# Grandediw/Unmanned_Aerial_Vehicles

Hardware: AMD Instinct MI355X
Metric: GP predictions/sec (mean+var) at N_train=65536, D=9 (higher is better)
Workload: dtype f32; 1 GPU; C3: N_train=65536, D=9, P=3, batched predict mean+var over 10000 query points per GPU per step (horizon 20 x 500 rollouts), fp32 predict on an fp64 factor; n_train=65536, features=9, outputs=3, parallelism=query-sharded x1, model replicated (every rank fits redundantly)

## Files before the change

### include/gpk.h

```cpp
#ifndef GPK_H
#define GPK_H

#include <stddef.h>
#include <stdint.h>

#ifdef __cplusplus
extern "C" {
#endif

typedef struct gpk_context* gpk_handle;

#define GPK_API __attribute__((visibility("default")))

enum { GPK_F32 = 0, GPK_F64 = 1 };
enum { GPK_OK = 0, GPK_NOT_PD = 1, GPK_BAD_ARG = 2, GPK_HIP_ERROR = 3 };
enum { GPK_TILE = 128, GPK_MAX_D = 64, GPK_MAX_D_PREDICT = 16, GPK_MAX_P = 16, GPK_MAX_BATCH = 8 };

GPK_API int gpk_create(gpk_handle* h, int device);
GPK_API void gpk_destroy(gpk_handle h);
GPK_API const char* gpk_last_error(gpk_handle h);
#define GPK_OWN_STREAM ((void*)(intptr_t)-1)
GPK_API int gpk_set_stream(gpk_handle h, void* stream);
GPK_API int gpk_synchronize(gpk_handle h);
GPK_API int64_t gpk_padded(int64_t n);
// ... 25 lines not shown

GPK_API int gpk_factor_to_f32(gpk_handle h, const double* L, int64_t Np, int64_t ldl, const double* winv,
                      float* Lf, int64_t ldlf, float* winvf);

GPK_API int gpk_potrs(gpk_handle h, const double* L, int64_t Np, int64_t ldl, const double* winv,
              const double* Y, int64_t N, int P, double* alpha);

GPK_API int gpk_potrs_inv(gpk_handle h, const double* W, int64_t Np, int64_t ldw, const double* Y, int64_t N,
                  int P, double* alpha);

GPK_API int gpk_trsm_lower_left(gpk_handle h, int dtype, const void* L, int64_t Np, int64_t ldl,
                        const void* winv, void* B, int64_t Mp, int64_t ldb);
GPK_API int gpk_colsumsq(gpk_handle h, int dtype, const void* B, int64_t Np, int64_t Mp, int64_t ldb,
                 double* out);

GPK_API int gpk_predict_mean(gpk_handle h, int dtype, const void* X, const void* alpha, int64_t N, int D,
                     int P, const double* ls, double sf2, const double* y_mean,
                     const double* y_std, const void* Xq, int64_t M, void* mean);

#define GPK_HOST_MAX_M 4096
GPK_API int gpk_predict_host(gpk_handle h, const double* X, const double* alpha, int64_t N, int D, int P,
                     const double* ls, double sf2, const double* y_mean, const double* y_std,
                     const double* W, int64_t Np, int64_t ldw, double kss, double floor_,
                     const double* Xq_host, int64_t M, double* mean_host, double* var_host);

GPK_API int gpk_predict_host_multi(gpk_handle h, int B, const double* const* X, const double* const* alpha, int64_t N, int D,
                           const double* ls, const double* sf2, const double* y_mean, const double* y_std,
                           const double* const* W, int64_t Np, int64_t ldw, const double* kss, double floor_,
                           const double* Xq_host, int64_t M, double* mean_host, double* var_host);

GPK_API int gpk_predict_mean_mfma(gpk_handle h, const float* X, const float* alpha, int64_t N, int D, int P,
                          const double* ls, double sf2, const double* center, const double* y_mean,
                          const double* y_std, const float* Xq, int64_t M, float* mean);

GPK_API int gpk_split3(gpk_handle h, const float* src, int64_t rows, int64_t cols, int64_t ld, void* dst);
GPK_API int gpk_predict_var_inv_split(gpk_handle h, const float* X, int64_t N, int D, const double* ls, double sf2,
                              const void* W3, int64_t Np, const float* Xq, int64_t M, double kss, double floor_,
                              float* work, void* work3, double* var);

GPK_API int gpk_split2_rows(gpk_handle h, const float* W, int64_t n, int64_t ld, float* scales, void* dst);
GPK_API int gpk_split2_rows_f64(gpk_handle h, const double* W, int64_t n, int64_t ld, float* scales, void* dst);
GPK_API int gpk_split2_rows_f64_absmax(gpk_handle h, const double* W, int64_t n, int64_t ld, float* scales, void* dst);
GPK_API int gpk_predict_var_inv_split2(gpk_handle h, const float* X, int64_t N, int D, const double* ls, double sf2,
                                       const void* W2, const float* w_scales, int64_t Np, const float* Xq, int64_t M,
                                       double kss, double floor_, void* work2, double* var);

GPK_API int gpk_predict_mean_var_split2(gpk_handle h, const float* X, const float* alpha, int64_t N, int D, int P,
                                        const double* ls, double sf2, const double* center, const double* y_mean,
                                        const double* y_std, const void* W2, const float* w_scales, int64_t Np,
                                        const float* Xq, int64_t M, double kss, double floor_, void* work2,
                                        float* mean_tmp, double recheck_below, unsigned* low_count, double* out);
GPK_API int gpk_pack_mean_var(gpk_handle h, int dtype, const void* mean, const double* var, int64_t M, int P,
                              const double* y_std, double* out);

GPK_API int gpk_predict_mean_multi(gpk_handle h, int dtype, const void* X, const void* alpha, int64_t N, int D,
                           int B, const double* ls, const double* sf2, const double* y_mean,
                           const double* y_std, const void* Xq, int64_t M, void* mean);

GPK_API int gpk_predict_var(gpk_handle h, int dtype, const void* X, int64_t N, int D, const double* ls,
                    double sf2, const void* L, int64_t Np, int64_t ldl, const void* winv,
                    const void* Xq, int64_t M, double kss, double floor, void* work,
                    double* var);

GPK_API int gpk_trtri(gpk_handle h, const double* L, int64_t Np, int64_t ldl, const double* winv, double* W,
              int64_t ldw, double* work);
GPK_API int gpk_trtri_absmax(gpk_handle h, const double* L, int64_t Np, int64_t ldl, const double* winv, double* W,
              int64_t ldw, double* work, float* block_absmax);
GPK_API int gpk_tril_to_f32(gpk_handle h, const double* A, int64_t Np, int64_t lda, float* Af, int64_t ldaf);
GPK_API int gpk_predict_var_inv(gpk_handle h, int dtype, const void* X, int64_t N, int D, const double* ls,
                        double sf2, const void* W, int64_t Np, int64_t ldw, const void* Xq, int64_t M,
                        double kss, double floor, void* work, double* var);

GPK_API int gpk_predict_cov_inv(gpk_handle h, int dtype, const void* X, int64_t N, int D, const double* ls, double sf2,
                                const void* W, int64_t Np, int64_t ldw, const void* Xq, int64_t M, double noise, void* work,
                                double* cov, int64_t ldc);
GPK_API int gpk_predict_cov(gpk_handle h, int dtype, const void* X, int64_t N, int D, const double* ls, double sf2,
                            const void* L, int64_t Np, int64_t ldl, const void* winv, const void* Xq, int64_t M, double noise,
                            void* work, double* cov, int64_t ldc);
GPK_API int gpk_predict_host_cov(gpk_handle h, const double* X, const double* alpha, int64_t N, int D, int P,
                                 const double* ls, double sf2, const double* y_mean, const double* y_std, const double* W,
                                 int64_t Np, int64_t ldw, double noise, const double* Xq_host, int64_t M, double* mean_host,
                                 double* cov_host);
GPK_API int gpk_predict_host_multi_cov(gpk_handle h, int B, const double* const* X, const double* const* alpha, int64_t N,
                                       int D, const double* ls, const double* sf2, const double* y_mean, const double* y_std,
                                       const double* const* W, int64_t Np, int64_t ldw, const double* noise,
                                       const double* Xq_host, int64_t M, double* mean_host, double* cov_host);
GPK_API int gpk_predict_batched_cov(gpk_handle h, const double* Xq, int64_t M, double* mean, double* cov);

GPK_API int gpk_predict_mean_grad(gpk_handle h, const double* X, const double* alpha, int64_t N, int D, int P, const double* ls,
                                  double sf2, const double* y_std, const double* Xq, int64_t M, double* dmean);
GPK_API int gpk_predict_var_grad_inv(gpk_handle h, const double* X, int64_t N, int D, const double* ls, double sf2,
                                     const double* W, int64_t Np, int64_t ldw, const double* Xq, int64_t M, double kss,
                                     double floor, double* work, double* var, double* dvar);
GPK_API int gpk_predict_host_grad(gpk_handle h, const double* X, const double* alpha, int64_t N, int D, int P, const double* ls,
                                  double sf2, const double* y_mean, const double* y_std, const double* W, int64_t Np,
                                  int64_t ldw, double kss, double floor, const double* Xq_host, int64_t M, double* mean_host,
                                  double* var_host, double* dmean_host, double* dvar_host);
GPK_API int gpk_predict_model_grad(gpk_handle h, const double* Xq, int64_t M, double* mean, double* var, double* dmean,
                                   double* dvar, int var_includes_noise);
GPK_API int gpk_predict_host_multi_grad(gpk_handle h, int B, const double* const* X, const double* const* alpha, int64_t N,
                                        int D, const double* ls, const double* sf2, const double* y_mean, const double* y_std,
                                        const double* const* W, int64_t Np, int64_t ldw, const double* kss, double floor,
                                        const double* Xq_host, int64_t M, double* mean_host, double* var_host,
                                        double* dmean_host, double* dvar_host);
GPK_API int gpk_predict_mean_grad_multi(gpk_handle h, const double* X, const double* alpha, int64_t N, int D, int B,
                                        const double* ls, const double* sf2, const double* y_std, const double* Xq, int64_t M,
// ... 264 lines not shown
```

### unmanned_aerial_vehicles_amd/_build.py

```python
import os
import shutil
import subprocess

PKG_DIR = os.path.dirname(os.path.abspath(__file__))
CSRC = os.path.join(PKG_DIR, "csrc")
LIB_PATH = os.path.join(PKG_DIR, "libgpk.so")
SOURCES = ["gpk_api.hip", "gpk_gram.hip", "gpk_gemm.hip", "gpk_chol.hip", "gpk_ptile.hip", "gpk_grad.hip", "gpk_mean.hip", "gpk_k5split.hip", "gpk_small.hip",
           "gpk_cov.hip", "gpk_jac.hip", "gpk_hess.hip", "gpk_serve.hip", "gpk_model.hip", "gpk_bmodel.hip", "gpk_sparse.hip", "gpk_select.hip", "gpk_paths.hip",
           "gpk_propagate.hip", "gpk_moments.hip"]
FLAGS = ["--offload-arch=gfx950", "-O3", "-std=c++17", "-fPIC", "-fvisibility=hidden", "-Wall", "-Wno-unused-function"]


def _stale():
    if not os.path.exists(LIB_PATH):
        return True
    t = os.path.getmtime(LIB_PATH)
    deps = [os.path.join(CSRC, f) for f in os.listdir(CSRC)] + [
        os.path.join(os.path.dirname(PKG_DIR), "include", "gpk.h")]
    return any(os.path.getmtime(d) > t for d in deps)


def build(force=False, verbose=False, extra_flags=(), variant=None):
    if variant is None and not force and not _stale():
        return LIB_PATH
    hipcc = shutil.which("hipcc") or "/opt/rocm/bin/hipcc"
    if not os.path.exists(hipcc):
        raise RuntimeError("hipcc not found: cannot build libgpk.so")
    objdir = os.path.join(PKG_DIR, "build") if variant is None else os.path.join(PKG_DIR, "build", "var_" + variant)
    lib_path = LIB_PATH if variant is None else os.path.join(PKG_DIR, "build", f"libgpk_{variant}.so")
    os.makedirs(objdir, exist_ok=True)
    objs = []
    procs = []
    for src in SOURCES:
        obj = os.path.join(objdir, src.replace(".hip", ".o"))
        cmd = [hipcc, *FLAGS, *extra_flags, "-c", os.path.join(CSRC, src), "-o", obj]
        procs.append((src, subprocess.Popen(cmd, stdout=subprocess.PIPE, stderr=subprocess.STDOUT, text=True)))
        objs.append(obj)
    for src, p in procs:
        out, _ = p.communicate()
        if verbose and out:
            print(out)
        if p.returncode != 0:
            raise RuntimeError(f"hipcc failed on {src}:\n{out}")
    tmp = lib_path + ".tmp"
    cmd = [hipcc, "--offload-arch=gfx950", "-shared", "-fPIC", "-o", tmp, *objs]
    r = subprocess.run(cmd, stdout=subprocess.PIPE, stderr=subprocess.STDOUT, text=True)
    if r.returncode != 0:
        raise RuntimeError(f"link failed:\n{r.stdout}")
    os.replace(tmp, lib_path)
    return lib_path


if __name__ == "__main__":
    import sys
    if len(sys.argv) > 1:
        print(build(variant=sys.argv[1], extra_flags=tuple(sys.argv[2:]), verbose=True))
    else:
        print(build(force=True, verbose=True))
```

### unmanned_aerial_vehicles_amd/_lib.py

```python
import ctypes as C
import os

import numpy as np

from ._build import LIB_PATH

GPK_F32, GPK_F64 = 0, 1
GPK_OK, GPK_NOT_PD, GPK_BAD_ARG, GPK_HIP_ERROR = 0, 1, 2, 3
GPK_TILE, GPK_MAX_D, GPK_MAX_P = 128, 64, 16
GPK_HOST_MAX_M = 4096
GPK_TIMED_K5, GPK_TIMED_GRAM, GPK_TIMED_GRAD, GPK_TIMED_POTRF = 1, 2, 3, 4
GPK_TIMED_COV = 5
GPK_TIMED_JAC = 6
GPK_TIMED_SPARSE_STATS, GPK_TIMED_SPARSE_PASS = 7, 8
GPK_TIMED_PROPAGATE = 9

_vp, _i64, _int, _dbl = C.c_void_p, C.c_int64, C.c_int, C.c_double
_dp = C.POINTER(C.c_double)
_f64 = np.dtype(np.float64)

SIGNATURES = {
    "gpk_create": (_int, [C.POINTER(_vp), _int]),
    "gpk_destroy": (None, [_vp]),
    "gpk_last_error": (C.c_char_p, [_vp]),
    "gpk_set_stream": (_int, [_vp, _vp]),
    "gpk_synchronize": (_int, [_vp]),
    "gpk_padded": (_i64, [_i64]),
    "gpk_fit": (_int, [_vp, _dp, _i64, _int, _dp, _int, _dp, _int, _dbl, _dbl, _dbl, _int]),
    "gpk_predict": (_int, [_vp, _vp, _i64, _vp, _vp, _int, _int]),
    "gpk_lml": (_int, [_vp, _dp, _int, _dp, _dp]),
    "gpk_fit_batched": (_int, [_vp, _int, _dp, _i64, _int, _dp, _dp, _int, _dp, _dp, _dbl, _int, C.POINTER(C.c_int)]),
    "gpk_predict_batched": (_int, [_vp, _dp, _i64, _dp, _dp, _int]),
    "gpk_lml_batched": (_int, [_vp, _dp, _int, _dp, _dp]),
    "gpk_export": (_int, [_vp, C.POINTER(_i64), C.POINTER(_int), C.POINTER(_int), _dp, _dp, _dp, _dp, _dp]),
    "gpk_import": (_int, [_vp, _dp, _i64, _int, _dp, _dp, _int, _dp, _int, _dbl, _dbl, _dp, _dp]),
    "gpk_model_release": (_int, [_vp]),
    "gpk_split2_rows": (_int, [_vp, _vp, _i64, _i64, _vp, _vp]),
    "gpk_split2_rows_f64": (_int, [_vp, _vp, _i64, _i64, _vp, _vp]),
    "gpk_split2_rows_f64_absmax": (_int, [_vp, _vp, _i64, _i64, _vp, _vp]),
    "gpk_predict_var_inv_split2": (_int, [_vp, _vp, _i64, _int, _dp, _dbl, _vp, _vp, _i64, _vp, _i64, _dbl, _dbl, _vp, _vp]),
    "gpk_predict_mean_var_split2": (_int, [_vp, _vp, _vp, _i64, _int, _int, _dp, _dbl, _dp, _dp, _dp, _vp, _vp, _i64, _vp, _i64,
                                           _dbl, _dbl, _vp, _vp, _dbl, _vp, _vp]),
    "gpk_pack_mean_var": (_int, [_vp, _int, _vp, _vp, _i64, _int, _dp, _vp]),
    "gpk_set_option": (_int, [_vp, C.c_char_p, _int]),
    "gpk_set_option_str": (_int, [_vp, C.c_char_p, C.c_char_p]),
    "gpk_timing": (_int, [_vp, _int]),
    "gpk_kernel_times": (_int, [_vp, _int, _dp, _int, C.POINTER(_int)]),
    "gpk_batch_begin": (_int, [_vp, _int]),
    "gpk_batch_buffer": (_int, [_vp, _vp, _i64]),
    "gpk_batch_end": (_int, [_vp]),
    "gpk_version": (C.c_char_p, []),
    "gpk_gram": (_int, [_vp, _int, _vp, _i64, _int, _dp, _dbl, _dbl, _vp, _i64]),
    "gpk_gram_rows": (_int, [_vp, _int, _vp, _i64, _int, _dp, _dbl, _dbl, _i64, _i64, _vp, _i64]),
    "gpk_cross_gram_t": (_int, [_vp, _int, _vp, _i64, _vp, _i64, _int, _dp, _dbl, _vp, _i64]),
    "gpk_rbf_kernel_grad": (_int, [_vp, _vp, _i64, _vp, _i64, _int, _dp, _dbl, _vp, _vp, _i64]),
    "gpk_potrf": (_int, [_vp, _vp, _i64, _i64, _vp, C.POINTER(_int)]),
    "gpk_leaf_inverses": (_int, [_vp, _vp, _i64, _i64, _vp]),
    "gpk_factor_to_f32": (_int, [_vp, _vp, _i64, _i64, _vp, _vp, _i64, _vp]),
    "gpk_potrs": (_int, [_vp, _vp, _i64, _i64, _vp, _vp, _i64, _int, _vp]),
    "gpk_potrs_inv": (_int, [_vp, _vp, _i64, _i64, _vp, _i64, _int, _vp]),
    "gpk_wtw": (_int, [_vp, _vp, _i64, _i64, _vp, _i64]),
    "gpk_trsm_lower_left": (_int, [_vp, _int, _vp, _i64, _i64, _vp, _vp, _i64, _i64]),
    "gpk_colsumsq": (_int, [_vp, _int, _vp, _i64, _i64, _i64, _vp]),
    "gpk_predict_mean": (_int, [_vp, _int, _vp, _vp, _i64, _int, _int, _dp, _dbl, _dp, _dp, _vp, _i64, _vp]),
    "gpk_split3": (_int, [_vp, _vp, _i64, _i64, _i64, _vp]),
    "gpk_predict_var_inv_split": (_int, [_vp, _vp, _i64, _int, _dp, _dbl, _vp, _i64, _vp, _i64, _dbl, _dbl, _vp, _vp, _vp]),
    "gpk_predict_host": (_int, [_vp, _vp, _vp, _i64, _int, _int, _vp, _dbl, _vp, _vp, _vp, _i64, _i64, _dbl, _dbl, _vp,
                                _i64, _vp, _vp]),
    "gpk_predict_host_multi": (_int, [_vp, _int, _vp, _vp, _i64, _int, _vp, _vp, _vp, _vp, _vp, _i64, _i64, _vp, _dbl, _vp,
                                      _i64, _vp, _vp]),
    "gpk_predict_mean_mfma": (_int, [_vp, _vp, _vp, _i64, _int, _int, _dp, _dbl, _dp, _dp, _dp, _vp, _i64, _vp]),
    "gpk_predict_mean_multi": (_int, [_vp, _int, _vp, _vp, _i64, _int, _int, _dp, _dp, _dp, _dp, _vp, _i64, _vp]),
    "gpk_predict_var": (_int, [_vp, _int, _vp, _i64, _int, _dp, _dbl, _vp, _i64, _i64, _vp, _vp, _i64, _dbl,
                               _dbl, _vp, _vp]),
    "gpk_trtri": (_int, [_vp, _vp, _i64, _i64, _vp, _vp, _i64, _vp]),
    "gpk_trtri_absmax": (_int, [_vp, _vp, _i64, _i64, _vp, _vp, _i64, _vp, _vp]),
    "gpk_tril_to_f32": (_int, [_vp, _vp, _i64, _i64, _vp, _i64]),
    "gpk_predict_var_inv": (_int, [_vp, _int, _vp, _i64, _int, _dp, _dbl, _vp, _i64, _i64, _vp, _i64, _dbl, _dbl,
                                   _vp, _vp]),
    "gpk_predict_cov_inv": (_int, [_vp, _int, _vp, _i64, _int, _dp, _dbl, _vp, _i64, _i64, _vp, _i64, _dbl, _vp, _vp,
                                   _i64]),
    "gpk_predict_cov": (_int, [_vp, _int, _vp, _i64, _int, _dp, _dbl, _vp, _i64, _i64, _vp, _vp, _i64, _dbl, _vp, _vp,
                               _i64]),
    "gpk_predict_host_cov": (_int, [_vp, _vp, _vp, _i64, _int, _int, _vp, _dbl, _vp, _vp, _vp, _i64, _i64, _dbl, _vp, _i64,
                                    _vp, _vp]),
    "gpk_predict_model_cov": (_int, [_vp, _dp, _i64, _dp, _dp]),
    "gpk_predict_host_multi_cov": (_int, [_vp, _int, _vp, _vp, _i64, _int, _vp, _vp, _vp, _vp, _vp, _i64, _i64, _vp, _vp, _i64,
                                          _vp, _vp]),
    "gpk_predict_batched_cov": (_int, [_vp, _dp, _i64, _dp, _dp]),
    "gpk_predict_mean_grad": (_int, [_vp, _vp, _vp, _i64, _int, _int, _dp, _dbl, _dp, _vp, _i64, _vp]),
    "gpk_predict_var_grad_inv": (_int, [_vp, _vp, _i64, _int, _dp, _dbl, _vp, _i64, _i64, _vp, _i64, _dbl, _dbl, _vp, _vp, _vp]),
    "gpk_predict_host_grad": (_int, [_vp, _vp, _vp, _i64, _int, _int, _vp, _dbl, _vp, _vp, _vp, _i64, _i64, _dbl, _dbl, _vp,
                                     _i64, _vp, _vp, _vp, _vp]),
    "gpk_predict_model_grad": (_int, [_vp, _dp, _i64, _dp, _dp, _dp, _dp, _int]),
    "gpk_predict_host_multi_grad": (_int, [_vp, _int, _vp, _vp, _i64, _int, _vp, _vp, _vp, _vp, _vp, _i64, _i64, _vp, _dbl, _vp,
                                           _i64, _vp, _vp, _vp, _vp]),
    "gpk_predict_mean_grad_multi": (_int, [_vp, _vp, _vp, _i64, _int, _int, _dp, _dp, _dp, _vp, _i64, _vp]),
    "gpk_predict_batched_grad": (_int, [_vp, _dp, _i64, _dp, _dp, _dp, _dp, _int]),
    "gpk_predict_mean_hess": (_int, [_vp, _vp, _vp, _i64, _int, _int, _dp, _dbl, _dp, _vp, _i64, _vp]),
    "gpk_predict_host_hess": (_int, [_vp, _vp, _vp, _i64, _int, _int, _vp, _dbl, _vp, _vp, _vp, _i64, _vp, _vp, _vp]),
    "gpk_predict_host_multi_hess": (_int, [_vp, _int, _vp, _vp, _i64, _int, _vp, _vp, _vp, _vp, _vp, _i64, _vp, _vp, _vp]),
    "gpk_predict_mean_hess_multi": (_int, [_vp, _vp, _vp, _i64, _int, _int, _dp, _dp, _dp, _vp, _i64, _vp]),
    "gpk_predict_model_hess": (_int, [_vp, _dp, _i64, _dp, _dp, _dp]),
    "gpk_predict_batched_hess": (_int, [_vp, _dp, _i64, _dp, _dp, _dp]),
    "gpk_sparse_predict_hess": (_int, [_vp, _dp, _i64, _dp, _dp, _dp]),
    "gpk_sparse_predict_multi_hess": (_int, [_vp, _int, C.POINTER(_vp), _dp, _i64, _dp, _dp, _dp]),
    "gpk_lml_terms": (_int, [_vp, _vp, _i64, _i64, _vp, _vp, _int, _dp]),
    "gpk_potri": (_int, [_vp, _vp, _i64, _i64, _vp, _vp, _i64, _vp]),
    "gpk_lml_grad": (_int, [_vp, _vp, _i64, _int, _dp, _dbl, _dbl, _vp, _int, _vp, _i64, _dp]),
    "gpk_lml_eval": (_int, [_vp, _vp, _i64, _int, _dp, _dbl, _dbl, _dbl, _vp, _int, _vp, _i64, _vp, _vp, _vp, _vp, _vp, _dp, _dp,
                            C.POINTER(C.c_int)]),
    "gpk_sparse_accumulate": (_int, [_vp, _vp, _vp, _i64, _vp, _i64, _int, _int, _dp, _dbl, _vp, _i64]),
    "gpk_sparse_grad_pass": (_int, [_vp, _vp, _vp, _i64, _vp, _i64, _int, _int, _dp, _dbl, _vp, _i64, _vp]),
    "gpk_sparse_zgrad_pass": (_int, [_vp, _vp, _vp, _i64, _vp, _i64, _int, _int, _dp, _dbl, _vp, _i64, _vp]),
    "gpk_sparse_hold": (_int, [_vp, _dp, _dp, _i64]),
    "gpk_sparse_eval": (_int, [_vp, _dp, _int, _dbl, _dbl, _dp, _dp, C.POINTER(_int)]),
    "gpk_sparse_eval_z": (_int, [_vp, _dp, _dp, _int, _dbl, _dbl, _dp, _dp, _dp, C.POINTER(_int)]),
    "gpk_greedy_select_bytes": (C.c_size_t, [_i64, _i64]),
    "gpk_greedy_select": (_int, [_vp, _vp, _i64, _int, _dp, _int, _dbl, _i64, _dbl, _dbl, _vp, _vp, _vp, _vp, _vp]),
    "gpk_sparse_select": (_int, [_vp, _dp, _i64, _i64, _dbl, _dbl, C.POINTER(_i64), _dp, _dp, C.POINTER(_i64)]),
    "gpk_sparse_begin": (_int, [_vp, _dp, _i64, _int, _int, _dp, _int, _dbl, _dbl, _dbl, _dbl, _dp, _dp]),
    "gpk_sparse_update": (_int, [_vp, _dp, _dp, _i64]),
    "gpk_sparse_finalize": (_int, [_vp, C.POINTER(_int)]),
    "gpk_sparse_predict": (_int, [_vp, _dp, _i64, _dp, _dp, _int]),
# ... 108 lines not shown
```

### unmanned_aerial_vehicles_amd/device.py

```python
from __future__ import annotations

import ctypes as C
import os
import threading

import numpy as np

from . import _lib
from ._lib import GPK_F32, GPK_F64, GPKError, NotPositiveDefinite
from .propagate import horizon_call

_backends = {}
_backends_lock = threading.Lock()


_torch_module = None


def _torch():
    global _torch_module
    if _torch_module is None:
        import torch
        _torch_module = torch
    return _torch_module


class Backend:

    def __init__(self, device_index=0):
        torch = _torch()
        self.lib = _lib.load()
        if not torch.cuda.is_available():
            raise RuntimeError("no HIP device visible: the GP kernels need an MI355X (there is no CPU fallback)")
        self.device_index = int(device_index)
        self.device = torch.device("cuda", self.device_index)
        torch.cuda.set_device(self.device)
        h = C.c_void_p()
        rc = self.lib.gpk_create(C.byref(h), self.device_index)
        if rc != _lib.GPK_OK:
            raise GPKError(rc, "gpk_create failed")
        self.h = h
        self.lock = threading.RLock()
        self.options = {}
        if os.environ.get("GPK_DEBUG_FILL"):
            self.check(self.lib.gpk_set_option(self.h, b"debug_fill", 1))
        self.bind_stream()
        self.low_count = torch.zeros((1,), dtype=torch.int32, device=self.device)
        self.low_seen = 0

    def bind_stream(self):
        rc = self.lib.gpk_set_stream(self.h, _torch().cuda.current_stream(self.device).cuda_stream)
        if rc:
            self.check(rc)

    def check(self, rc):
        if rc == _lib.GPK_OK:
            return
        msg = self.lib.gpk_last_error(self.h).decode()
        if rc == _lib.GPK_NOT_PD:
            raise NotPositiveDefinite(msg)
        raise GPKError(rc, msg)

    def status(self, name, *args):
        with self.lock:
            self.bind_stream()
            return getattr(self.lib, name)(self.h, *args)

    def call(self, name, *args):
        with self.lock:
            self.bind_stream()
            rc = getattr(self.lib, name)(self.h, *args)
            if rc:
                self.check(rc)
        return rc

    def close(self):
        h, self.h = self.h, None
        if h:
            self.lib.gpk_destroy(h)

    def sync(self):
        self.check(self.lib.gpk_synchronize(self.h))

    def set_options(self, **opts):
        for k, v in opts.items():
            if isinstance(v, str):
                self.check(self.lib.gpk_set_option_str(self.h, k.encode(), v.encode()))
            else:
                self.check(self.lib.gpk_set_option(self.h, k.encode(), int(v)))
            self.options[k] = v
        return self

    def empty(self, shape, dtype):
        t = _torch().empty(shape, dtype=dtype, device=self.device)
        if os.environ.get("GPK_DEBUG_FILL"):
            t.fill_(float(os.environ["GPK_DEBUG_FILL"]) if t.is_floating_point() else 255)
        return t

    def upload(self, a, dtype=None):
        torch = _torch()
# ... 387 lines not shown
                "dtypes": {"X": "float64", "alpha": "float64", "W2": "uint8", "w_scales": "float32"}}
        return meta, {"X": self.X, "alpha": self.alpha, "W2": W2, "w_scales": w_scales}

    @classmethod
    def from_serving_state(cls, meta, tensors, backend=None):
        torch = _torch()
        self = cls.__new__(cls)
        self.be = backend or get_backend()
        self.N, self.D, self.P, self.Np = int(meta["N"]), int(meta["D"]), int(meta["P"]), int(meta["Np"])
        self.X = tensors["X"]
        self._Xh = self.X.cpu().numpy()
        self._xc = self._Xh.mean(axis=0)
        self._r2 = {}
        self.Yn = None
        self.K = self.winv = None
        self.alpha = tensors["alpha"]
        self.factored = True
        self.ls = np.ascontiguousarray(meta["ls"], dtype=np.float64)
        self.sf2 = float(meta["sf2"])
        self._f32 = None
        self._Winv = {"split2": (tensors["W2"], tensors["w_scales"])}
        self._host_args = None
        self._amp = self._alpha_sq = None
        self._Kinv = None
        self.replica = True
        return self

    FP32_MEAN_ERR_PER_AMP = {"mfma": 7.0e-7, "valu": 1.1e-6}
    FP32_MEAN_TOL = 1e-4
    FP32_BATCH_GATE_ROWS = 1024
    FP32_BATCH_GATE_MARGIN = 1.3
    FP32_VAR_RECHECK_FRACTION = 1e-2

    def _amplification_at(self, q64):
        zeros, ones = np.zeros(self.P), np.ones(self.P)
        sq = getattr(self, "_alpha_sq", None)
        if sq is None:
            sq = self._alpha_sq = self.alpha ** 2
        b = self.predict_mean_dev(q64, zeros, ones, "float64", "valu").abs().amax(dim=0)
        a2 = self.predict_mean_dev(q64, zeros, ones, "float64", "valu", _alpha=sq,
                                   _kernel=(self.ls / np.sqrt(2.0), self.sf2 ** 2)).amax(dim=0).sqrt()
        return float((a2 / b.clamp_min(1e-300)).max())

    def fp32_mean_amplification(self):
        torch = _torch()
        c = getattr(self, "_amp", None)
        if c is not None and c[0] is self.ls:
            return c[1]
        idx = torch.linspace(0, self.N - 1, min(self.N, 1024), device=self.be.device).round().long()
        amp = self._amplification_at(self.X[idx].contiguous())
        self._amp = (self.ls, amp)
        return amp

    def fp32_mean_ok(self, q=None):
        torch = _torch()
        c = self.FP32_MEAN_ERR_PER_AMP[self.mean_kernel_choice()]
        if c * self.fp32_mean_amplification() <= self.FP32_MEAN_TOL:
            return True
        if q is None or len(q) == 0:
            return False
        M = len(q)
        if isinstance(q, torch.Tensor):
            idx = torch.linspace(0, M - 1, min(M, self.FP32_BATCH_GATE_ROWS), device=q.device).round().long()
            qs = q[idx].to(device=self.be.device, dtype=torch.float64).contiguous()
        else:
            idx = np.round(np.linspace(0, M - 1, min(M, self.FP32_BATCH_GATE_ROWS))).astype(np.int64)
            qs = self.be.upload(np.ascontiguousarray(np.asarray(q, dtype=np.float64)[idx]))
        return c * self.FP32_BATCH_GATE_MARGIN * self._amplification_at(qs) <= self.FP32_MEAN_TOL

    def predict_var_dev(self, Xq, kss, floor=0.0, dtype="float64", method="auto"):
        torch = _torch()
        assert self.factored
        f32 = dtype in ("float32", np.float32, torch.float32)
        if method == "auto":
            method = "inverse_split2" if f32 else "inverse"
        if method not in ("solve", "inverse", "inverse_split", "inverse_split2"):
            raise ValueError("method must be 'auto', 'solve', 'inverse', 'inverse_split' or 'inverse_split2'")
        if method in ("inverse_split", "inverse_split2") and not f32:
            raise ValueError("inverse_split / inverse_split2 are fp32 serving forms (bf16x3 / fp16x2 operand splits)")
        tdt = torch.float32 if f32 else torch.float64
        es = 4 if f32 else 8
        code = GPK_F32 if f32 else GPK_F64
        q = self._as_queries(Xq, tdt)
        M = q.shape[0]
        out = self.be.empty((M,), torch.float64)
        if M == 0:
            return out
        Xd = self._f32_data()["X"] if f32 else self.X
        if method == "inverse_split":
            W3 = self.split_inverse_factor()
        elif method == "inverse_split2":
            W2, w_scales = self.split2_inverse_factor()
        elif method == "inverse":
            Wd = self.inverse_factor(f32)
        elif f32:
            c = self._f32_factor()
            Ld, wd = c["L"], c["winv"]
        else:
            Ld, wd = self.K, self.winv
        panel = self._panel_rows(self.Np * es, M)
        work = self.be.empty((self.Np * panel,), tdt) if method != "inverse_split2" else None
        work3 = (self.be.empty((self.Np * panel * (6 if method == "inverse_split" else 4),), torch.uint8)
                 if method in ("inverse_split", "inverse_split2") else None)
        var = self.be.empty((panel,), torch.float64)
        be = self.be
        lsp = _hp(self.ls)
        with be.lock:
            for m0 in range(0, M, panel):
                m1 = min(M, m0 + panel)
                if method == "inverse_split":
                    be.call("gpk_predict_var_inv_split", _p(Xd), self.N, self.D, lsp, self.sf2, _p(W3), self.Np, _p(q[m0:m1]),
                            m1 - m0, float(kss), float(floor), _p(work), _p(work3), _p(var))
                elif method == "inverse_split2":
                    be.call("gpk_predict_var_inv_split2", _p(Xd), self.N, self.D, lsp, self.sf2, _p(W2), _p(w_scales), self.Np,
                            _p(q[m0:m1]), m1 - m0, float(kss), float(floor), _p(work3), _p(var))
                elif method == "inverse":
                    be.call("gpk_predict_var_inv", code, _p(Xd), self.N, self.D, lsp, self.sf2, _p(Wd), self.Np, self.Np,
                            _p(q[m0:m1]), m1 - m0, float(kss), float(floor), _p(work), _p(var))
                else:
                    be.call("gpk_predict_var", code, _p(Xd), self.N, self.D, lsp, self.sf2, _p(Ld), self.Np, self.Np, _p(wd),
                            _p(q[m0:m1]), m1 - m0, float(kss), float(floor), _p(work), _p(var))
# ... 182 lines not shown
    def moments_host(self, y_mean, y_std, kss, floor, Xq, Sq):
        M, nx = Xq.shape[0], Sq.shape[1]
        mean, cov, xcov = np.empty((M, self.P)), np.empty((M, self.P, self.P)), np.empty((M, self.P, self.D))
        self._moments_call("gpk_moments_host", y_mean, y_std, float(kss), float(floor), 0, 0.0, nx, _hp(Xq), _hp(Sq), M, _hp(mean),
                           _hp(cov), _hp(xcov))
        return mean, cov, xcov

    def propagate_mm_host(self, y_mean, y_std, kss, floor, x0, U, lin, S0, Q, R, H, stages):
        P, D = self.P, self.D
        traj, Sigma, more = horizon_call(
            lambda *t: self._moments_call("gpk_propagate_mm_host", y_mean, y_std, float(kss), float(floor), 0, 0.0, *t),
            x0, U, lin, S0, Q, R, H, ((P,), (P, P), (P, D)) if stages else None)
        return (traj, Sigma, *more)

    def _rows64(self, Xq, q, rows):
        torch = _torch()
        if isinstance(Xq, torch.Tensor):
            return Xq[rows.to(Xq.device)].to(device=self.be.device, dtype=torch.float64).contiguous()
        return self.be.upload(np.ascontiguousarray(np.asarray(Xq, dtype=np.float64)[rows.cpu().numpy()]))

    def _fp64_var_method(self):
        if self.replica:
            raise RuntimeError("a serving replica holds no factor: fp64 variances are computed on the rank that fitted the model")
        return "inverse" if ("f64" in self._Winv or self.Np <= self.INVERSE_EAGER_NP) else "solve"

    def _gate_mean(self, dtype, var_method, gated, q=None, mean_gate=None):
        torch = _torch()
        f32 = dtype in ("float32", np.float32, torch.float32)
        if f32 and gated and not (self.fp32_mean_ok(q) if mean_gate is None else mean_gate):
            return "float64", ("auto" if var_method in ("inverse_split", "inverse_split2") else var_method)
        return ("float32" if f32 else "float64"), var_method

    def predict_gated_dev(self, Xq, y_mean, y_std, kss=None, floor=0.0, dtype="float64", var_method="auto", gated=True,
                          mean_gate=None):
        torch = _torch()
        pd, vm = self._gate_mean(dtype, var_method, gated, Xq, mean_gate)
        q = self._as_queries(Xq, torch.float32 if pd == "float32" else torch.float64)
        mean = self.predict_mean_dev(q, y_mean, y_std, pd)
        if kss is None:
            return mean, None
        var = self.predict_var_dev(q, kss, floor, pd, vm)
        if gated and pd == "float32" and q.shape[0]:
            self._recheck_low_variances(Xq, q, var, kss, floor)
        return mean, var

    def _recheck_low_variances(self, Xq, q, var, kss, floor):
        low = _torch().nonzero(var < self.FP32_VAR_RECHECK_FRACTION * kss).ravel()
        if low.numel():
            var[low] = self.predict_var_dev(self._rows64(Xq, q, low), kss, floor, "float64", self._fp64_var_method())

    def predict_packed_dev(self, Xq, y_mean, y_std, kss, floor=0.0, dtype="float32", var_method="auto", gated=True,
                           mean_gate=None):
        torch = _torch()
        pd, vm = self._gate_mean(dtype, var_method, gated, Xq, mean_gate)
        f32 = pd == "float32"
        if vm == "auto":
            vm = "inverse_split2" if f32 else "inverse"
        q = self._as_queries(Xq, torch.float32 if f32 else torch.float64)
        M = q.shape[0]
        out = self.be.empty((M, 2 * self.P), torch.float64)
        if M == 0:
            return out
        ym, ys = _vec(y_mean, self.P), _vec(y_std, self.P)
        be = self.be
        if not (f32 and vm == "inverse_split2"):
            mean = self.predict_mean_dev(q, ym, ys, pd)
            var = self.predict_var_dev(q, kss, floor, pd, vm)
            if gated and f32:
                self._recheck_low_variances(Xq, q, var, kss, floor)
            be.call("gpk_pack_mean_var", GPK_F32 if f32 else GPK_F64, _p(mean), _p(var), M, self.P, _hp(ys), _p(out))
            return out
        c = self._f32_data()
        W2, w_scales = self.split2_inverse_factor()
        center = _hp(self._xc) if self.mean_kernel_choice() == "mfma" else None
        panel = self._panel_rows(self.Np * 4, M)
        work2 = be.empty((self.Np * panel * 4,), torch.uint8)
        mean_tmp = be.empty((panel * self.P,), torch.float32)
        thr = self.FP32_VAR_RECHECK_FRACTION * kss if gated else 0.0
        nlow = 0
        with be.lock:
            try:
                for m0 in range(0, M, panel):
                    m1 = min(M, m0 + panel)
                    be.call("gpk_predict_mean_var_split2", _p(c["X"]), _p(c["alpha"]), self.N, self.D, self.P, _hp(self.ls),
                            self.sf2, center, _hp(ym), _hp(ys), _p(W2), _p(w_scales), self.Np, _p(q[m0:m1]), m1 - m0,
                            float(kss), float(floor), _p(work2), _p(mean_tmp), float(thr),
                            _p(be.low_count) if gated else None, _p(out[m0:m1]))
            finally:
                if gated:
                    seen = int(be.low_count.item()) & 0xFFFFFFFF
                    nlow = (seen - be.low_seen) & 0xFFFFFFFF
                    be.low_seen = seen
        if nlow and not self.replica:
            ys2 = torch.as_tensor(ys ** 2, device=be.device)
            low = torch.nonzero(out[:, self.P] <= thr * float(ys[0] ** 2) * (1.0 + 1e-12)).ravel()
            v64 = self.predict_var_dev(self._rows64(Xq, q, low), kss, floor, "float64", self._fp64_var_method())
            out[low, self.P:] = v64[:, None] * ys2[None, :]
        return out

    def gram_host(self, ls, sf2, diag_add):
        self.gram(ls, sf2, diag_add)
        return self.K[: self.N, : self.N].cpu().numpy()


def prior_cov(X, ls, sf2, noise, device=None):
    torch = _torch()
    be = get_backend(device)
    X = np.ascontiguousarray(X, dtype=np.float64)
    M, D = X.shape
    if M == 0:
        return np.zeros((0, 0))
    if not 1 <= D <= _lib.GPK_MAX_D:
        raise ValueError(f"D must be in [1, {_lib.GPK_MAX_D}]")
    Mp = padded(M)
    q = be.upload(X)
    K = be.empty((Mp, Mp), torch.float64)
    be.call("gpk_gram", GPK_F64, _p(q), M, D, _hp(_vec(ls, D)), float(sf2), float(noise), _p(K), Mp)
    return K[:M, :M].cpu().numpy()
```

Baseline: 105,400 predictions/s.

## Speculate fp32 predict with fused on-device mean gate, fall back to fp64

Adds a dedicated HIP kernel that computes the batch fp32-mean amplification gate on device (sampled query rows, split-N partial sums plus a finish reduction) and writes the result into a shared word buffer alongside the low-variance counter. predict_packed_dev now queues this gate ahead of the fp32 split2 predict and reads gate result and low count in a single host sync, instead of running the gate synchronously before choosing a precision. If the gate fails, the whole batch is recomputed in fp64. This is meant to remove a blocking host round-trip and the separate amplification path, at the cost of wasted fp32 work whenever the gate rejects.

New measurement: 105,500 predictions/s, median of 2. No clear change (+0.1%).

```diff
diff --git a/include/gpk.h b/include/gpk.h
--- a/include/gpk.h
+++ b/include/gpk.h
@@ -101,6 +101,10 @@
                                         float* mean_tmp, double recheck_below, unsigned* low_count, double* out);
 GPK_API int gpk_pack_mean_var(gpk_handle h, int dtype, const void* mean, const double* var, int64_t M, int P,
                               const double* y_std, double* out);
+
+GPK_API int gpk_mean_gate(gpk_handle h, const double* X, const double* alpha, int64_t N, int D, int P, const double* ls,
+                          double sf2, int q_dtype, const void* Xq, int64_t M, double c_margin, double tol, void* out,
+                          int64_t* rows_out);
 
 GPK_API int gpk_predict_mean_multi(gpk_handle h, int dtype, const void* X, const void* alpha, int64_t N, int D,
                            int B, const double* ls, const double* sf2, const double* y_mean,
diff --git a/unmanned_aerial_vehicles_amd/_build.py b/unmanned_aerial_vehicles_amd/_build.py
--- a/unmanned_aerial_vehicles_amd/_build.py
+++ b/unmanned_aerial_vehicles_amd/_build.py
@@ -5,7 +5,7 @@
 PKG_DIR = os.path.dirname(os.path.abspath(__file__))
 CSRC = os.path.join(PKG_DIR, "csrc")
 LIB_PATH = os.path.join(PKG_DIR, "libgpk.so")
-SOURCES = ["gpk_api.hip", "gpk_gram.hip", "gpk_gemm.hip", "gpk_chol.hip", "gpk_ptile.hip", "gpk_grad.hip", "gpk_mean.hip", "gpk_k5split.hip", "gpk_small.hip",
+SOURCES = ["gpk_api.hip", "gpk_gram.hip", "gpk_gemm.hip", "gpk_chol.hip", "gpk_ptile.hip", "gpk_grad.hip", "gpk_mean.hip", "gpk_gate.hip", "gpk_k5split.hip", "gpk_small.hip",
            "gpk_cov.hip", "gpk_jac.hip", "gpk_hess.hip", "gpk_serve.hip", "gpk_model.hip", "gpk_bmodel.hip", "gpk_sparse.hip", "gpk_select.hip", "gpk_paths.hip",
            "gpk_propagate.hip", "gpk_moments.hip"]
 FLAGS = ["--offload-arch=gfx950", "-O3", "-std=c++17", "-fPIC", "-fvisibility=hidden", "-Wall", "-Wno-unused-function"]
diff --git a/unmanned_aerial_vehicles_amd/_lib.py b/unmanned_aerial_vehicles_amd/_lib.py
--- a/unmanned_aerial_vehicles_amd/_lib.py
+++ b/unmanned_aerial_vehicles_amd/_lib.py
@@ -70,6 +70,7 @@
     "gpk_predict_host_multi": (_int, [_vp, _int, _vp, _vp, _i64, _int, _vp, _vp, _vp, _vp, _vp, _i64, _i64, _vp, _dbl, _vp,
                                       _i64, _vp, _vp]),
     "gpk_predict_mean_mfma": (_int, [_vp, _vp, _vp, _i64, _int, _int, _dp, _dbl, _dp, _dp, _dp, _vp, _i64, _vp]),
+    "gpk_mean_gate": (_int, [_vp, _vp, _vp, _i64, _int, _int, _dp, _dbl, _int, _vp, _i64, _dbl, _dbl, _vp, _vp]),
     "gpk_predict_mean_multi": (_int, [_vp, _int, _vp, _vp, _i64, _int, _int, _dp, _dp, _dp, _dp, _vp, _i64, _vp]),
     "gpk_predict_var": (_int, [_vp, _int, _vp, _i64, _int, _dp, _dbl, _vp, _i64, _i64, _vp, _vp, _i64, _dbl,
                                _dbl, _vp, _vp]),
diff --git a/unmanned_aerial_vehicles_amd/csrc/gpk_gate.hip b/unmanned_aerial_vehicles_amd/csrc/gpk_gate.hip
--- /dev/null
+++ b/unmanned_aerial_vehicles_amd/csrc/gpk_gate.hip
@@ -0,0 +1,192 @@
+#include "gpk_internal.h"
+#include "gpk_math.h"
+
+namespace {
+
+constexpr int GT_QR = 2;
+constexpr int GT_ROWS = 1024;
+constexpr int GT_BLOCKS = 1024;
+
+struct Gate16 { double v[16]; };
+
+__device__ __forceinline__ long long gate_row(int s, long long M, int S) {
+  if (S <= 1) return 0;
+  const float end = (float)(M - 1);
+  const float step = end / (float)(S - 1);
+  float v;
+  if (s < S / 2) v = __fmul_rn(step, (float)s);
+  else v = __builtin_fmaf(-step, (float)(S - s - 1), end);
+  long long r = (long long)rintf(v);
+  return r < 0 ? 0 : (r > M - 1 ? M - 1 : r);
+}
+
+__device__ __forceinline__ double max_nan(double a, double b) { return (a > b || a != a) ? a : b; }
+
+template <int D4, int P4>
+__global__ __launch_bounds__(256) void mean_gate_kernel(const double* __restrict__ X, const double* __restrict__ alpha, long long N,
+                                                        int D, int P, Gate16 inv_ls, const void* __restrict__ Xq, int q_f32,
+                                                        long long M, int S, long long chunk, double* __restrict__ partial,
+                                                        long long* __restrict__ rows_out) {
+  constexpr int DD = 4 * D4, PP = 4 * P4, NV = GT_QR * 2 * PP;
+  __shared__ double xq_s[GT_QR][DD];
+  __shared__ double red[4][NV];
+  const int tid = threadIdx.x, lane = tid & 63, wave = tid >> 6;
+  const int s0 = blockIdx.x * GT_QR;
+  if (tid < GT_QR * DD) {
+    const int r = tid / DD, d = tid - r * DD, s = s0 + r;
+    double v = 0.0;
+    if (s < S && d < D) {
+      const long long row = gate_row(s, M, S);
+      v = q_f32 ? (double)static_cast<const float*>(Xq)[row * D + d] : static_cast<const double*>(Xq)[row * D + d];
+    }
+    xq_s[r][d] = v;
+  }
+  if (rows_out && blockIdx.y == 0 && tid < GT_QR && s0 + tid < S) rows_out[s0 + tid] = gate_row(s0 + tid, M, S);
+  __syncthreads();
+  double xq[GT_QR][DD];
+#pragma unroll
+  for (int r = 0; r < GT_QR; ++r)
+#pragma unroll
+    for (int d = 0; d < DD; ++d) xq[r][d] = xq_s[r][d];
+  double acc[GT_QR][2][PP];
+#pragma unroll
+  for (int r = 0; r < GT_QR; ++r)
+#pragma unroll
+    for (int p = 0; p < PP; ++p) acc[r][0][p] = acc[r][1][p] = 0.0;
+
+  const long long n0 = (long long)blockIdx.y * chunk;
+  const long long n1 = min(N, n0 + chunk);
+  for (long long j = n0 + tid; j < n1; j += 256) {
+    double xt[DD], al[PP];
+#pragma unroll
+    for (int d = 0; d < DD; ++d) xt[d] = d < D ? X[j * D + d] : 0.0;
+#pragma unroll
+    for (int p = 0; p < PP; ++p) al[p] = p < P ? alpha[j * P + p] : 0.0;
+#pragma unroll
+    for (int r = 0; r < GT_QR; ++r) {
+      double d2 = 0.0;
+#pragma unroll
+      for (int d = 0; d < DD; ++d) {
+        const double df = (xq[r][d] - xt[d]) * inv_ls.v[d];
+        d2 = __builtin_fma(df, df, d2);
+      }
+      const double k = gpk_exp_neg(-0.5 * d2);
+      const double k2 = k * k;
+#pragma unroll
+      for (int p = 0; p < PP; ++p) {
+        acc[r][0][p] = __builtin_fma(k, al[p], acc[r][0][p]);
+        acc[r][1][p] = __builtin_fma(k2, al[p] * al[p], acc[r][1][p]);
+      }
+    }
+  }
+
+#pragma unroll
+  for (int r = 0; r < GT_QR; ++r)
+#pragma unroll
+    for (int w = 0; w < 2; ++w)
+#pragma unroll
+      for (int p = 0; p < PP; ++p) {
+        double v = acc[r][w][p];
+#pragma unroll
+        for (int m = 32; m >= 1; m >>= 1) v += __shfl_xor(v, m, 64);
+        if (lane == 0) red[wave][(r * 2 + w) * PP + p] = v;
+      }
+  __syncthreads();
+  if (tid < NV) {
+    const int r = tid / (2 * PP), w = (tid / PP) & 1, p = tid % PP, s = s0 + r;
+    if (s < S && p < P)
+      partial[(((long long)blockIdx.y * S + s) * 2 + w) * P + p] = ((red[0][tid] + red[1][tid]) + red[2][tid]) + red[3][tid];
+  }
+}
+
+__global__ __launch_bounds__(256) void mean_gate_finish_kernel(const double* __restrict__ partial, int slices, int S, int P,
+                                                               double sf2, double c_margin, double tol, double* __restrict__ out) {
+  __shared__ double rb[256], ra[256];
+  const int tid = threadIdx.x;
+  double amp = 0.0;
+  for (int p = 0; p < P; ++p) {
+    double b = 0.0, a = 0.0;
+    for (int s = tid; s < S; s += 256) {
+      double s1 = 0.0, s2 = 0.0;
+      for (int c = 0; c < slices; ++c) {
+        const double* row = partial + (((long long)c * S + s) * 2) * P;
+        s1 += row[p];
+        s2 += row[P + p];
+      }
+      b = max_nan(b, fabs(sf2 * s1));
+      a = max_nan(a, (sf2 * sf2) * s2);
+    }
+    rb[tid] = b; ra[tid] = a;
+    __syncthreads();
+    for (int h = 128; h >= 1; h >>= 1) {
+      if (tid < h) { rb[tid] = max_nan(rb[tid], rb[tid + h]); ra[tid] = max_nan(ra[tid], ra[tid + h]); }
+      __syncthreads();
+    }
+    if (tid == 0) amp = max_nan(amp, sqrt(ra[0]) / max_nan(rb[0], 1e-300));
+    __syncthreads();
+  }
+  if (tid == 0) {
+    out[0] = amp;
+    reinterpret_cast<int*>(out)[2] = (c_margin * amp <= tol) ? 1 : 0;
+  }
+}
+
+typedef void (*gate_fn)(const double*, const double*, long long, int, int, Gate16, const void*, int, long long, int, long long,
+                        double*, long long*);
+template <int D4>
+gate_fn gate_pick_p(int p4) {
+  switch (p4) {
+    case 1: return mean_gate_kernel<D4, 1>;
+    case 2: return mean_gate_kernel<D4, 2>;
+    case 3: return mean_gate_kernel<D4, 3>;
+    default: return mean_gate_kernel<D4, 4>;
+  }
+}
+gate_fn gate_pick(int d4, int p4) {
+  switch (d4) {
+    case 1: return gate_pick_p<1>(p4);
+    case 2: return gate_pick_p<2>(p4);
+    case 3: return gate_pick_p<3>(p4);
+    default: return gate_pick_p<4>(p4);
+  }
+}
+}
+
+extern "C" int gpk_mean_gate(gpk_handle h, const double* X, const double* alpha, int64_t N, int D, int P, const double* ls,
+                             double sf2, int q_dtype, const void* Xq, int64_t M, double c_margin, double tol, void* out,
+                             int64_t* rows_out) {
+  if (!h) return GPK_BAD_ARG;
+  GPK_REQUIRE(h, X && alpha && ls && Xq && out, "mean_gate: null pointer");
+  GPK_REQUIRE(h, N >= 1 && M >= 1, "mean_gate: empty input");
+  GPK_REQUIRE(h, D >= 1 && D <= 16, "mean_gate: D must be in [1, 16]");
+  GPK_REQUIRE(h, P >= 1 && P <= 16, "mean_gate: P must be in [1, 16]");
+  GPK_REQUIRE(h, q_dtype == GPK_F32 || q_dtype == GPK_F64, "mean_gate: bad query dtype");
+  GPK_REQUIRE(h, ((uintptr_t)out & 7) == 0, "mean_gate: out must be 8-byte aligned");
+  Gate16 inv{};
+  for (int d = 0; d < D; ++d) {
+    GPK_REQUIRE(h, ls[d] > 0.0, "mean_gate: length-scales must be positive");
+    inv.v[d] = 1.0 / ls[d];
+  }
+  const int S = (int)(M < GT_ROWS ? M : GT_ROWS);
+  const int nbx = (S + GT_QR - 1) / GT_QR;
+  int64_t slices = GT_BLOCKS / nbx;
+  const int64_t max_slices = (N + 255) / 256;
+  if (slices > max_slices) slices = max_slices;
+  if (slices < 1) slices = 1;
+  int64_t chunk = (N + slices - 1) / slices;
+  chunk = (chunk + 255) / 256 * 256;
+  slices = (N + chunk - 1) / chunk;
+  if (h->gram_log)
+    fprintf(stderr, "GPKGATE %s %lld %lld %d %d rows%d grid%dx%lld chunk%lld\n", q_dtype == GPK_F64 ? "f64" : "f32", (long long)N,
+            (long long)M, D, P, S, nbx, (long long)slices, (long long)chunk);
+  void* partial = nullptr;
+  GPK_TRY(gpk_scratch(h, (size_t)slices * S * 2 * P * sizeof(double), &partial));
+  hipLaunchKernelGGL(gate_pick((D + 3) / 4, (P + 3) / 4), dim3((unsigned)nbx, (unsigned)slices), dim3(256), 0, h->stream, X, alpha,
+                     (long long)N, D, P, inv, Xq, q_dtype == GPK_F32 ? 1 : 0, (long long)M, S, (long long)chunk, (double*)partial,
+                     (long long*)rows_out);
+  GPK_LAUNCH_CHECK(h);
+  hipLaunchKernelGGL(mean_gate_finish_kernel, dim3(1), dim3(256), 0, h->stream, (const double*)partial, (int)slices, S, P, sf2,
+                     c_margin, tol, (double*)out);
+  GPK_LAUNCH_CHECK(h);
+  return GPK_OK;
+}
diff --git a/unmanned_aerial_vehicles_amd/device.py b/unmanned_aerial_vehicles_amd/device.py
--- a/unmanned_aerial_vehicles_amd/device.py
+++ b/unmanned_aerial_vehicles_amd/device.py
@@ -45,7 +45,8 @@
         if os.environ.get("GPK_DEBUG_FILL"):
             self.check(self.lib.gpk_set_option(self.h, b"debug_fill", 1))
         self.bind_stream()
-        self.low_count = torch.zeros((1,), dtype=torch.int32, device=self.device)
+        self.gate_words = torch.zeros((4,), dtype=torch.int32, device=self.device)
+        self.low_count = self.gate_words[3:]
         self.low_seen = 0
 
     def bind_stream(self):
@@ -539,21 +540,46 @@
         self._amp = (self.ls, amp)
         return amp
 
+    def _model_mean_ok(self):
+        c = self.FP32_MEAN_ERR_PER_AMP[self.mean_kernel_choice()]
+        return c * self.fp32_mean_amplification() <= self.FP32_MEAN_TOL
+
+    def queue_batch_gate(self, q, rows_out=None):
+        torch = _torch()
+        be = self.be
+        M = len(q)
+        if not (isinstance(q, torch.Tensor) and q.device == be.device and q.dtype in (torch.float32, torch.float64)
+                and q.is_contiguous()):
+            if isinstance(q, torch.Tensor):
+                idx = torch.linspace(0, M - 1, min(M, self.FP32_BATCH_GATE_ROWS), device=q.device).round().long()
+                q = q[idx].to(device=be.device, dtype=torch.float64).contiguous()
+            else:
+                idx = np.round(np.linspace(0, M - 1, min(M, self.FP32_BATCH_GATE_ROWS))).astype(np.int64)
+                q = be.upload(np.ascontiguousarray(np.asarray(q, dtype=np.float64)[idx]))
+            M = q.shape[0]
+        if q.ndim != 2 or q.shape[1] != self.D:
+            raise ValueError(f"queries must be (M, {self.D})")
+        c = self.FP32_MEAN_ERR_PER_AMP[self.mean_kernel_choice()]
+        be.call("gpk_mean_gate", _p(self.X), _p(self.alpha), self.N, self.D, self.P, _hp(self.ls), self.sf2,
+                GPK_F32 if q.dtype == torch.float32 else GPK_F64, _p(q), M, c * self.FP32_BATCH_GATE_MARGIN, self.FP32_MEAN_TOL,
+                _p(be.gate_words), _p(rows_out))
+
+    def read_batch_gate(self):
+        w = self.be.gate_words.cpu().numpy()
+        return float(w[:2].view(np.float64)[0]), bool(w[2]), int(w[3]) & 0xFFFFFFFF
+
+    def fp32_batch_amplification(self, q, rows_out=None):
+        with self.be.lock:
+            self.queue_batch_gate(q, rows_out)
+            a2, ok, _ = self.read_batch_gate()
+        return a2, ok
+
     def fp32_mean_ok(self, q=None):
-        torch = _torch()
-        c = self.FP32_MEAN_ERR_PER_AMP[self.mean_kernel_choice()]
-        if c * self.fp32_mean_amplification() <= self.FP32_MEAN_TOL:
+        if self._model_mean_ok():
             return True
         if q is None or len(q) == 0:
             return False
-        M = len(q)
-        if isinstance(q, torch.Tensor):
-            idx = torch.linspace(0, M - 1, min(M, self.FP32_BATCH_GATE_ROWS), device=q.device).round().long()
-            qs = q[idx].to(device=self.be.device, dtype=torch.float64).contiguous()
-        else:
-            idx = np.round(np.linspace(0, M - 1, min(M, self.FP32_BATCH_GATE_ROWS))).astype(np.int64)
-            qs = self.be.upload(np.ascontiguousarray(np.asarray(q, dtype=np.float64)[idx]))
-        return c * self.FP32_BATCH_GATE_MARGIN * self._amplification_at(qs) <= self.FP32_MEAN_TOL
+        return self.fp32_batch_amplification(q)[1]
 
     def predict_var_dev(self, Xq, kss, floor=0.0, dtype="float64", method="auto"):
         torch = _torch()
@@ -842,6 +868,11 @@
     def predict_packed_dev(self, Xq, y_mean, y_std, kss, floor=0.0, dtype="float32", var_method="auto", gated=True,
                            mean_gate=None):
         torch = _torch()
+        speculate = False
+        if (mean_gate is None and gated and dtype in ("float32", np.float32, torch.float32)
+                and var_method in ("auto", "inverse_split2") and len(Xq)):
+            speculate = not self._model_mean_ok()
+            mean_gate = True
         pd, vm = self._gate_mean(dtype, var_method, gated, Xq, mean_gate)
         f32 = pd == "float32"
         if vm == "auto":
@@ -868,8 +899,11 @@
         mean_tmp = be.empty((panel * self.P,), torch.float32)
         thr = self.FP32_VAR_RECHECK_FRACTION * kss if gated else 0.0
         nlow = 0
+        gate_ok = True
         with be.lock:
             try:
+                if speculate:
+                    self.queue_batch_gate(Xq)
                 for m0 in range(0, M, panel):
                     m1 = min(M, m0 + panel)
                     be.call("gpk_predict_mean_var_split2", _p(c["X"]), _p(c["alpha"]), self.N, self.D, self.P, _hp(self.ls),
@@ -878,9 +912,14 @@
                             _p(be.low_count) if gated else None, _p(out[m0:m1]))
             finally:
                 if gated:
-                    seen = int(be.low_count.item()) & 0xFFFFFFFF
+                    if speculate:
+                        _, gate_ok, seen = self.read_batch_gate()
+                    else:
+                        seen = int(be.low_count.item()) & 0xFFFFFFFF
                     nlow = (seen - be.low_seen) & 0xFFFFFFFF
                     be.low_seen = seen
+        if not gate_ok:
+            return self.predict_packed_dev(Xq, y_mean, y_std, kss, floor, "float64", "auto", gated)
         if nlow and not self.replica:
             ys2 = torch.as_tensor(ys ** 2, device=be.device)
             low = torch.nonzero(out[:, self.P] <= thr * float(ys[0] ** 2) * (1.0 + 1e-12)).ravel()
```
